# r4dl/LAENeRF

Hardware: AMD Instinct MI355X
Metric: Mrays/s, lego 800x800 train-step (4096 rays/step) (higher is better)
Workload: dtype f16 (table, MLP) / f32 (march, composite); 1 GPU; configs[1]: lego-like 800x800 pinhole rays, 4096 random pixels of one view per step, L=16 T=2^19 F=2 hash grid + 2x64 / 3x64 ffmlp, cascade 1, analytic occupancy (13% occupied), steady-state train step incl. backward + Adam; hip_graph_replay=True, march_pipelined_on_side_stream=True, steps_per_graph_replay=4, parallelism=1 independent ray-batch replicas (no data-path collective)

## Files before the change

### include/laenerf.h

```cpp
#ifndef LAENERF_H
#define LAENERF_H

#include <stdint.h>

#ifdef __cplusplus
extern "C" {
#endif

#if defined(__GNUC__) || defined(__clang__)
#define LAE_API __attribute__((visibility("default")))
#else
#define LAE_API
#endif

#define LAE_OK 0
#define LAE_EINVAL (-1)
#define LAE_ELAUNCH (-2)
#define LAE_ENULL (-3)

#define LAE_F32 0
#define LAE_F16 1

#define LAE_GRID_HASH 0
#define LAE_GRID_TILED 1
#define LAE_INTERP_LINEAR 0
#define LAE_INTERP_SMOOTHSTEP 1

#define LAE_ACT_RELU 0
#define LAE_ACT_EXPONENTIAL 1
#define LAE_ACT_SINE 2
#define LAE_ACT_SIGMOID 3
#define LAE_ACT_SQUAREPLUS 4
#define LAE_ACT_SOFTPLUS 5
#define LAE_ACT_NONE 6

#define LAE_ABI_TAG "abi16"
LAE_API const char* lae_version(void);
LAE_API const char* lae_last_error(void);


LAE_API int lae_near_far_from_aabb(const float* rays_o, const float* rays_d, const float* aabb,
                           uint32_t N, float min_near, float* nears, float* fars, void* stream);

LAE_API int lae_get_rays(const float* poses, uint32_t B, float fx, float fy, float cx, float cy, uint32_t H, uint32_t W,
                 const int64_t* inds, uint64_t inds_batch_stride, uint32_t N, int perturb, float off_x, float off_y,
                 float* rays_o, float* rays_d, const float* aabb, float min_near, float* nears, float* fars, void* stream);

#define LAE_IMG_U8 0
#define LAE_IMG_F16 1
#define LAE_IMG_F32 2
#define LAE_BATCH_IMAGE 0
#define LAE_BATCH_ALL 1
#define LAE_BG_WHITE 0
#define LAE_BG_RANDOM 1
LAE_API int lae_sample_train_batch(const void* images, int dtype, uint32_t n_img, uint32_t H, uint32_t W, uint32_t C,
                           const float* poses, float fx, float fy, float cx, float cy, uint32_t N,
                           const float* aabb, float min_near, uint64_t seed, int64_t* step_counter, int mode, int bg_mode,
                           int srgb_to_linear, float* rays_o, float* rays_d, float* nears, float* fars, float* gt,
                           float* bg_out, int64_t* inds, void* stream);
// ... 153 lines not shown
                                const int32_t* offsets_host, int32_t* nonfinite_flag, uint32_t* touched_lines, uint32_t* grad_dirty,
                                void* stream);

LAE_API uint64_t lae_grid_backward_plan_bytes(uint32_t B, uint32_t L);
LAE_API uint64_t lae_grid_touched_lines_words(uint64_t n_entries);
LAE_API int lae_grid_encode_backward_plan(const float* inputs, const int32_t* offsets, uint32_t B, uint32_t D, uint32_t C, uint32_t L,
                                  float S, uint32_t H, uint32_t gridtype, int align_corners, uint32_t interp, int dtype,
                                  float in_shift, float in_scale, const int32_t* offsets_host, void* plan,
                                  uint32_t* touched_lines, void* stream);
LAE_API int lae_grid_encode_backward_planned(const void* grad, const float* inputs, const int32_t* offsets, void* grad_embeddings,
                                     uint32_t B, uint32_t D, uint32_t C, uint32_t L, float S, uint32_t H, uint32_t gridtype,
                                     int align_corners, uint32_t interp, int dtype, float in_shift, float in_scale,
                                     const int32_t* offsets_host, const void* plan, int32_t* nonfinite_flag, uint32_t* grad_dirty,
                                     void* stream);

LAE_API uint64_t lae_grid_backward_workspace_bytes(uint32_t B, uint32_t L, int dtype);

LAE_API int lae_grid_forward_schedule(const int32_t* offsets_host, uint32_t L, float S, uint32_t H, uint32_t n_chunks,
                              uint32_t* nseg_out, uint32_t* segs_out);

LAE_API int lae_grid_set_forward_mode(int mode);

LAE_API int lae_grid_set_backward_mode(int mode);

LAE_API int lae_grad_total_variation(const void* inputs, const void* embeddings, void* grad,
                             const int32_t* offsets, float weight, uint32_t B, uint32_t D,
                             uint32_t C, uint32_t L, float S, uint32_t H, uint32_t gridtype,
                             int align_corners, int dtype, void* stream);


LAE_API int lae_sh_encode_forward(const float* inputs, float* outputs, uint32_t B, uint32_t D,
                          uint32_t C, float* dy_dx, void* stream);

LAE_API int lae_sh_encode_backward(const float* grad, const float* inputs, uint32_t B, uint32_t D,
                           uint32_t C, const float* dy_dx, float* grad_inputs, void* stream);


LAE_API int lae_ffmlp_forward(const void* inputs, const void* weights, uint32_t B, uint32_t input_dim,
                      uint32_t output_dim, uint32_t hidden_dim, uint32_t num_layers,
                      uint32_t activation, uint32_t output_activation, void* forward_buffer,
                      void* outputs, void* stream);

LAE_API int lae_ffmlp_inference(const void* inputs, const void* weights, uint32_t B, uint32_t input_dim,
                        uint32_t output_dim, uint32_t hidden_dim, uint32_t num_layers,
                        uint32_t activation, uint32_t output_activation, void* inference_buffer,
                        void* outputs, void* stream);
// ... 188 lines not shown
```

### laenerf_amd/_lib.py

```python
import ctypes
import os

import torch

_HERE = os.path.dirname(os.path.abspath(__file__))
SO_PATH = os.environ.get("LAE_HIP_LIB") or os.path.join(_HERE, "lib", "liblaenerf_hip.so")

u32, u64, f32, i32, vp = ctypes.c_uint32, ctypes.c_uint64, ctypes.c_float, ctypes.c_int, ctypes.c_void_p
i64, f64 = ctypes.c_int64, ctypes.c_double

SIGNATURES = {
    "lae_near_far_from_aabb": [vp, vp, vp, u32, f32, vp, vp, vp],
    "lae_sph_from_ray": [vp, vp, f32, u32, vp, vp],
    "lae_get_rays": [vp, u32, f32, f32, f32, f32, u32, u32, vp, u64, u32, i32, f32, f32, vp, vp, vp, f32, vp, vp, vp],
    "lae_morton3D": [vp, u32, vp, vp],
    "lae_morton3D_invert": [vp, u32, vp, vp],
    "lae_packbits": [vp, u32, f32, vp, vp],
    "lae_march_rays_train_scratch_bytes": [u32],
    "lae_march_rays_train": [vp, vp, vp, f32, f32, u32, u32, u32, u32, u32, vp, vp, vp, vp, vp, vp, vp, vp, vp, vp, vp],
    "lae_march_rays_train_limit": [vp, vp, vp, f32, f32, u32, u32, u32, u32, u32, vp, vp, vp, vp, vp, vp, vp, vp, vp, vp, vp, vp],
    "lae_sample_train_batch": [vp, i32, u32, u32, u32, u32, vp, f32, f32, f32, f32, u32, vp, f32, u64, vp, i32, i32, i32, vp, vp, vp, vp, vp,
                               vp, vp, vp],
    "lae_sample_train_batch_weighted": [vp, i32, u32, u32, u32, u32, vp, f32, f32, f32, f32, u32, vp, f32, u64, vp, i32, i32, vp, vp,
                                        vp, vp, vp, vp, vp, vp, vp, vp],
# ... 10 lines not shown
    "lae_march_rays": [u32, u32, vp, vp, vp, vp, f32, f32, u32, u32, u32, vp, vp, vp, vp, vp, vp, vp, vp],
    "lae_march_rays_distill": [u32, u32, vp, vp, vp, vp, f32, f32, u32, u32, u32, vp, vp, vp, vp, vp, vp, vp, vp, vp, vp],
    "lae_composite_rays": [u32, u32, f32, vp, vp, vp, vp, vp, vp, vp, vp, vp],
    "lae_composite_rays_distill": [u32, u32, f32, vp, vp, vp, vp, vp, vp, vp, vp, vp, vp, vp, vp],
    "lae_render_frame_workspace_bytes": [u32, u32, u64],
    "lae_render_frame_set_overlap": [i32],
    "lae_render_frame_mode": [],
    "lae_render_frame_last_status": [],
    "lae_render_frame_probe_us": [vp, u32],
    "lae_render_frame": [vp, vp, u32, vp, f32, vp, vp, f32, f32, u32, u32, u32, vp, vp, vp, u32, f32, u32, u32, i32, u32, vp, vp, f32, f32,
                         u32, u64, vp, vp, f32, f32, f32, i32, i32, vp, vp, vp, vp, vp, vp, u64, vp, vp],
    "lae_compact_scratch_bytes": [u32],
    "lae_compact_rays_alive": [vp, u32, vp, vp, vp, vp],
    "lae_grid_encode_forward": [vp, vp, vp, vp, u32, u32, u32, u32, f32, u32, vp, u32, i32, u32, i32, vp],
    "lae_grid_encode_backward": [vp, vp, vp, vp, vp, u32, u32, u32, u32, f32, u32, vp, vp, u32, i32, u32, i32, vp],
    "lae_grid_encode_forward_ex": [vp, vp, vp, vp, u32, u32, u32, u32, f32, u32, vp, u32, i32, u32, i32, i32, f32, f32, vp, vp],
    "lae_grid_encode_backward_ex": [vp, vp, vp, vp, vp, u32, u32, u32, u32, f32, u32, vp, vp, u32, i32, u32, i32, i32, f32, f32, vp, vp, vp, vp, vp],
    "lae_grid_backward_workspace_bytes": [u32, u32, i32],
    "lae_grid_backward_plan_bytes": [u32, u32],
    "lae_grid_touched_lines_words": [u64],
    "lae_grid_encode_backward_plan": [vp, vp, u32, u32, u32, u32, f32, u32, u32, i32, u32, i32, f32, f32, vp, vp, vp, vp],
    "lae_grid_encode_backward_planned": [vp, vp, vp, vp, u32, u32, u32, u32, f32, u32, u32, i32, u32, i32, f32, f32, vp, vp, vp, vp, vp],
    "lae_grid_set_backward_mode": [i32],
    "lae_grid_set_forward_mode": [i32],
    "lae_grid_forward_schedule": [vp, u32, f32, u32, u32, vp, vp],
    "lae_grad_total_variation": [vp, vp, vp, vp, f32, u32, u32, u32, u32, f32, u32, u32, i32, i32, vp],
    "lae_sh_encode_forward": [vp, vp, u32, u32, u32, vp, vp],
    "lae_sh_encode_backward": [vp, vp, u32, u32, u32, vp, vp, vp],
    "lae_freq_encode_forward": [vp, u32, u32, u32, u32, vp, vp],
    "lae_freq_encode_backward": [vp, vp, u32, u32, u32, u32, vp, vp],
    "lae_ffmlp_forward": [vp, vp, u32, u32, u32, u32, u32, u32, u32, vp, vp, vp],
    "lae_ffmlp_inference": [vp, vp, u32, u32, u32, u32, u32, u32, u32, vp, vp, vp],
    "lae_ffmlp_backward": [vp, vp, vp, vp, u32, u32, u32, u32, u32, u32, u32, i32, vp, vp, vp, vp],
    "lae_ffmlp_backward_ex": [vp, vp, vp, vp, u32, u32, u32, u32, u32, u32, u32, i32, vp, vp, vp, i32, vp, vp],
    "lae_nerf_head_forward": [vp, vp, vp, vp, u32, f32, vp, vp, vp, i32, vp],
    "lae_nerf_density_forward": [vp, vp, u32, f32, vp, vp, i32, vp],
    "lae_density_grid_positions": [vp, u32, u32, f32, vp, vp, vp, vp],
    "lae_density_grid_partial_scratch_bytes": [u32, u32],
    "lae_density_grid_partial_positions": [vp, u32, vp, vp, vp, u32, u32, f32, vp, vp, vp, vp, vp],
    "lae_density_grid_update": [vp, vp, u32, f32, f32, u32, vp, vp, vp],
    "lae_mark_untrained_grid": [vp, u32, f32, f32, f32, f32, u32, u32, f32, f32, i32, vp, vp],
    "lae_nerf_head_backward": [vp, vp, vp, vp, vp, vp, vp, vp, u32, f32, vp, vp, vp, vp, i32, i32, vp, vp, u32, u32, vp, vp, vp],
    "lae_nerf_field_backward": [vp, vp, vp, vp, vp, vp, vp, vp, u32, f32, vp, vp, vp, vp, i32, vp, vp, u32, u32, vp, vp,
                                vp, vp, vp, u32, f32, u32, u32, i32, u32, f32, f32, vp, vp, vp, vp, vp, vp],
    "lae_palette_forward": [vp, vp, vp, u32, u32, u32, vp, vp, vp, vp],
    "lae_palette_backward_scratch_bytes": [u32],
# ... 37 lines not shown
    "lae_workspace_bytes": [i32],
    "lae_version": [],
    "lae_last_error": [],
}
_RESTYPES = {
    "lae_march_rays_train_scratch_bytes": u64,
    "lae_compact_scratch_bytes": u64,
    "lae_density_grid_partial_scratch_bytes": u64,
    "lae_palette_backward_scratch_bytes": u64,
    "lae_style_loss_scratch_bytes": u64,
    "lae_recolor_compact_scratch_bytes": u64,
    "lae_marching_cubes_scratch_bytes": u64,
    "lae_style_image_scratch_bytes": u64,
    "lae_render_frame_workspace_bytes": u64,
    "lae_workspace_bytes": u64,
    "lae_grid_backward_workspace_bytes": u64,
    "lae_grid_backward_plan_bytes": u64,
    "lae_grid_touched_lines_words": u64,
    "lae_version": ctypes.c_char_p,
    "lae_last_error": ctypes.c_char_p,
}

_lib = None
ABI_TAG = b"abi16"


def _abi_of(path):
    lib = ctypes.CDLL(path)
    fn = lib.lae_version
    fn.argtypes, fn.restype = [], ctypes.c_char_p
    return lib, fn().split()[-1]


def load():
    global _lib
    if _lib is not None:
        return _lib
    if not os.path.exists(SO_PATH):
        raise RuntimeError(
            f"laenerf_amd: HIP library not built ({SO_PATH}); run `python -m laenerf_amd.build` "
            "(there is no CPU fallback)")
    if not os.environ.get("LAE_HIP_LIB"):
        from . import build as _build
        if _build.default_is_packed(SO_PATH):
            _build.build(force=True)
            if _build.default_is_packed(SO_PATH):
                raise RuntimeError(f"laenerf_amd: {SO_PATH} was built with packed-fp32 instructions and could not be rebuilt without them")
# ... 70 lines not shown
```

### laenerf_amd/backend.py

```python
import sys
import types

import numpy as np
import torch

from . import _lib
from ._lib import check, need_contig, need_cuda, ptr, stream

_F16 = torch.float16


def _dtype_code(t):
    if t.dtype == torch.float32:
        return 0
    if t.dtype == torch.float16:
        return 1
    raise RuntimeError(f"laenerf_amd: unsupported dtype {t.dtype} (float32 / float16 only)")


def _host_i32(a, n):
    if a is None:
        return None
    if not (isinstance(a, np.ndarray) and a.dtype == np.int32 and a.flags.c_contiguous and a.size == n):
        raise RuntimeError("laenerf_amd: offsets_host must be a contiguous int32 numpy array with L + 1 entries")
# ... 430 lines not shown
            check(lib.lae_grid_encode_backward_planned(ptr(grad), ptr(inputs), ptr(offsets), ptr(grad_embeddings), B, D, C, L, float(S), H,
                                                       gridtype, int(bool(align_corners)), interp, _dtype_code(grad), float(in_map[0]),
                                                       float(in_map[1]), _host_i32(offsets_host, L + 1), ptr(plan), nonfinite_flag, grad_dirty, stream()),
                  "grid_encode_backward")
            return
        args = (ptr(grad), ptr(inputs), ptr(embeddings), ptr(offsets), ptr(grad_embeddings), B, D, C, L, float(S), H,
                ptr(dy_dx), ptr(grad_inputs), gridtype, int(bool(align_corners)), interp, _dtype_code(grad))
        if (blc or tuple(in_map) != (0.0, 1.0) or offsets_host is not None or nonfinite_flag is not None or touched_lines is not None
                or grad_dirty is not None):
            check(lib.lae_grid_encode_backward_ex(*args, int(bool(blc)), float(in_map[0]), float(in_map[1]), _host_i32(offsets_host, L + 1),
                                                  nonfinite_flag, touched_lines, grad_dirty, stream()), "grid_encode_backward")
        else:
            check(lib.lae_grid_encode_backward(*args, stream()), "grid_encode_backward")

    @staticmethod
    def grid_backward_workspace_bytes(B, L, half=True):
        return int(_lib.load().lae_grid_backward_workspace_bytes(B, L, 1 if half else 0))

    @staticmethod
    def set_backward_mode(mode):
        check(_lib.load().lae_grid_set_backward_mode(int(mode)), "grid_set_backward_mode")

    @staticmethod
    def grad_total_variation(inputs, embeddings, grad, offsets, weight, B, D, C, L, S, H, gridtype, align_corners):
        need_cuda(inputs, embeddings, grad, offsets); need_contig(inputs, embeddings, grad, offsets)
        check(_lib.load().lae_grad_total_variation(ptr(inputs), ptr(embeddings), ptr(grad), ptr(offsets), float(weight), B, D,
                                                   C, L, float(S), H, gridtype, int(bool(align_corners)),
                                                   _dtype_code(embeddings), stream()), "grad_total_variation")


class _SHEncoder:
    @staticmethod
    def sh_encode_forward(inputs, outputs, B, D, C, dy_dx):
        need_cuda(inputs, outputs, dy_dx); need_contig(inputs, outputs, dy_dx)
        if inputs.dtype != torch.float32 or outputs.dtype != torch.float32:
            raise RuntimeError("sh_encode_forward: float32 required (sphere_harmonics.py:16 casts to fp32)")
        check(_lib.load().lae_sh_encode_forward(ptr(inputs), ptr(outputs), B, D, C, ptr(dy_dx), stream()), "sh_encode_forward")

    @staticmethod
    def sh_encode_backward(grad, inputs, B, D, C, dy_dx, grad_inputs):
        need_cuda(grad, inputs, dy_dx, grad_inputs); need_contig(grad, inputs, dy_dx, grad_inputs)
        if grad.dtype != torch.float32:
            raise RuntimeError("sh_encode_backward: float32 required")
        check(_lib.load().lae_sh_encode_backward(ptr(grad), ptr(inputs), B, D, C, ptr(dy_dx), ptr(grad_inputs), stream()),
              "sh_encode_backward")

# ... 350 lines not shown
        check(lib.lae_recolor_compact(ptr(depth), ptr(weights_sum), ptr(rays_o), ptr(rays_d), N, ptr(indices), ptr(slot_map), ptr(x_term),
                                      ptr(dirs), ptr(alpha), ptr(count), ptr(ws), stream()), "recolor_compact")

    @staticmethod
    def recolor_compose(slot_map, N, w_logits, o_raw, P, active_mask, palette, p_weights, p_bias, alpha, base, bg, mode, k, flags, out,
                        out_u8=None):
        ts = (slot_map, w_logits, o_raw, palette, p_weights, p_bias, alpha, base, bg, out, out_u8)
        need_cuda(*ts); need_contig(*ts)
        if w_logits.dtype != _F16 or o_raw.dtype != _F16 or slot_map.dtype != torch.int32 or (out_u8 is not None and out_u8.dtype != torch.uint8):
            raise RuntimeError("recolor_compose: logits / offsets float16, slot_map int32, out_u8 uint8")
        _need_f32(*(t for t in (palette, p_weights, p_bias, alpha, base, bg, out) if t is not None))
        if slot_map.numel() < N or out.numel() < 3 * N or (base is not None and base.numel() < 3 * N) or \
                (out_u8 is not None and out_u8.numel() < 3 * N) or bg.numel() < 3:
            raise RuntimeError("recolor_compose: a buffer is smaller than the view")
        check(_lib.load().lae_recolor_compose(ptr(slot_map), N, ptr(w_logits), w_logits.shape[1], ptr(o_raw), o_raw.shape[1], P, active_mask,
                                              ptr(palette), ptr(p_weights), ptr(p_bias), ptr(alpha), ptr(base), ptr(bg), int(mode), int(k),
                                              int(flags), ptr(out), ptr(out_u8), stream()), "recolor_compose")


style_backend = _Style

for _cls in (_RayMarching, _GridEncoder, _SHEncoder, _FFMLP):
    for _k, _v in list(vars(_cls).items()):
        if isinstance(_v, staticmethod) and not _k.startswith("_") and _k not in ("fused_backward_available", "ffmlp_set_mode", "set_backward_mode",
                                                                                   "allocate_splitk", "free_splitk", "render_frame_last_status",
                                                                                   "render_frame_check"):
            setattr(_cls, _k, staticmethod(_wrap_timed(_k, _v.__func__)))

raymarching_backend = _RayMarching
gridencoder_backend = _GridEncoder
shencoder_backend = _SHEncoder
ffmlp_backend = _FFMLP
freqencoder_backend = _FreqEncoder


def _as_module(name, cls):
    m = types.ModuleType(name)
    for k, v in vars(cls).items():
        if not k.startswith("_") and isinstance(v, staticmethod):
            setattr(m, k, v.__func__)
    m.__doc__ = f"laenerf_amd HIP backend standing in for the reference's `{name}` extension"
    return m


def install_as_reference_backends():
    _lib.load()
    for name, cls in (("_raymarching", _RayMarching), ("_gridencoder", _GridEncoder), ("_shencoder", _SHEncoder),
# ... 3 lines not shown
```

### laenerf_amd/csrc/gridencoder.hip

```cpp
#include <math.h>
#include <stdio.h>
#include <stdlib.h>
#include <algorithm>
#include <type_traits>
#include "lae_common.h"
#include "dw_reduce.h"
#include <vector>
#include <mutex>
#include <utility>

namespace {

constexpr int MAX_LEVELS = 32;
struct LevelScales { float scale[MAX_LEVELS]; float in_shift, in_scale; };

typedef _Float16 half_t;
typedef _Float16 half2_t __attribute__((ext_vector_type(2)));

__constant__ uint32_t k_primes[7] = {1u, 2654435761u, 805459861u, 3674653429u, 2097192037u, 1434869437u, 2165219737u};

#ifdef LAE_GRID_STAMPS
__device__ unsigned long long g_grid_stamps[32768 * 32];
#define GRID_STAMP(slot, i) do { if (threadIdx.x == 0 && (uint32_t)(i) < 32u) g_grid_stamps[(size_t)(slot) * 32 + (i)] = wall_clock64(); } while (0)
#define GRID_NOTE(slot, i, v) do { if (threadIdx.x == 0 && (uint32_t)(i) < 32u) g_grid_stamps[(size_t)(slot) * 32 + (i)] = (v); } while (0)
// ... 355 lines not shown
                    (__attribute__((address_space(1))) half2_t*)(tab + gi + ch), v);
            }
        } else {
#pragma unroll
            for (int ch = 0; ch < C; ch++) atomicAdd(tab + gi + ch, w * gc[ch]);
        }
    }
}

template <typename T> struct BVal;
template <> struct BVal<half_t> { using type = uint2; };
template <> struct BVal<float> { using type = float4; };
constexpr int FILL_THREADS = 256;
constexpr int SPT = 4;
constexpr int SEGS = 1;
constexpr uint32_t UNIT_SAMPLES = FILL_THREADS * SPT;
constexpr uint32_t STAGE_CAP = 4096 + 256;
constexpr uint32_t KEY_SINGLE = 15u;
constexpr int ACC_THREADS = 1024;
constexpr uint32_t BWD_MAX_SAMPLES = 1u << 24;
constexpr uint32_t COARSE_RES = 64;
constexpr bool WIDE_COARSE_UNITS = false;
constexpr uint32_t SUB_RECS = 64;
constexpr uint32_t TICKET_ARRIVALS = 2;
constexpr uint32_t TICKET_WORDS = TICKET_ARRIVALS + MAX_LEVELS * SUB_RECS;
template <typename T> constexpr uint32_t sub_rec_words() { return (sizeof(T) == 2 ? 2 * PART : PART) + PART / 64; }

struct BwdPlan {
    uint16_t* cnt;
    uint32_t* part_cnt;
    uint32_t* totals;
    uint32_t* offs;
    uint32_t* tickets;
};

__host__ __device__ __forceinline__ lae_dw::DwTailJob* plan_tail_job(const BwdPlan& plan) {
    static_assert((TICKET_WORDS * 4) % alignof(lae_dw::DwTailJob) == 0, "the tail job sits right behind the tickets");
    return reinterpret_cast<lae_dw::DwTailJob*>(plan.tickets + TICKET_WORDS);
}
__host__ __device__ __forceinline__ uint32_t* plan_dirty_snapshot(const BwdPlan& plan) {
    return plan.tickets + TICKET_WORDS + sizeof(lae_dw::DwTailJob) / 4;
}

__device__ __forceinline__ uint32_t pack_half2(float a, float b) {
    const half2_t h = {(half_t)a, (half_t)b};
    return __builtin_bit_cast(uint32_t, h);
// ... 381 lines not shown
}
__device__ __forceinline__ uint32_t fix24_to_half(long long t) {
    const uint32_t sign = t < 0 ? 0x8000u : 0u;
    const unsigned long long mag = t < 0 ? (unsigned long long)(-t) : (unsigned long long)t;
    if (mag < 1024ull) return sign | (uint32_t)mag;
    const int msb = 63 - __builtin_clzll(mag);
    const int shift = msb - 10;
    unsigned long long q = mag >> shift;
    if (shift > 0) {
        const unsigned long long rem = mag & ((1ull << shift) - 1ull), halfway = 1ull << (shift - 1);
        if (rem > halfway || (rem == halfway && (q & 1ull))) q++;
    }
    int e = msb - 9;
    if (q == 2048ull) { q = 1024ull; e++; }
    if (e >= 31) return sign | 0x7c00u;
    return sign | ((uint32_t)e << 10) | ((uint32_t)q & 1023u);
}
__device__ __forceinline__ bool half_nonfinite(uint32_t u) { return (u & 0x7c00u) == 0x7c00u; }

template <typename T>
__global__ __launch_bounds__(ACC_THREADS, 8) void k_bwd_acc(
    const int32_t* __restrict__ offsets, T* __restrict__ grad_grid, uint32_t L, LevelScales sc, uint32_t gridtype,
    bool align_corners, BwdPlan plan, const typename BVal<T>::type* __restrict__ qvals, const uint16_t* __restrict__ qkeys,
    unsigned long long* __restrict__ partials, int32_t* __restrict__ nf_flag, uint32_t bk_target) {
    using V = typename BVal<T>::type;
    constexpr bool HALF = sizeof(T) == 2;
    constexpr uint32_t ACCW = HALF ? 2 * PART : PART;
    __shared__ unsigned long long acc64[ACCW];
    __shared__ uint32_t poison[PART / 32];
    __shared__ uint32_t s_cnt[MAX_LEVELS], s_sub[MAX_LEVELS], s_first[MAX_LEVELS];
    __shared__ uint32_t s_ticket, s_arr;
    const uint32_t tid = threadIdx.x;
    if (tid < L) {
        const LevelBins lb = level_bins_of((uint32_t)(offsets[tid + 1] - offsets[tid]), bk_target);
        s_cnt[tid] = lb.P <= BK_MAX ? lb.P * lb.SUB : 0u;
        s_sub[tid] = lb.SUB;
    }
    __syncthreads();
    if (tid == 0) { uint32_t run = 0; for (uint32_t l = 0; l < L; l++) { s_first[l] = run; run += s_cnt[l]; } s_arr = run; }
    __syncthreads();
    const uint32_t total_buckets = s_arr;
    __syncthreads();

    auto apply = [&](uint32_t key, const V& v) {
        const uint32_t e0 = key & (PART - 1), code = key >> 12;
        const uint32_t e1 = e0 ^ ((2u << code) - 1u);
        if constexpr (HALF) {
            const uint32_t w0 = v.x, w1 = v.y;
            const uint32_t carry = (((w0 & 0x7c007c00u) + 0x28002800u) | ((w1 & 0x7c007c00u) + 0x28002800u)) & 0x80008000u;
            if (carry == 0) {
                long long a, b;
                half2_to_fix24_small(w0, a, b);
                atomicAdd(&acc64[e0], (unsigned long long)a);
                atomicAdd(&acc64[PART + e0], (unsigned long long)b);
// ... 2 lines not shown
                atomicAdd(&acc64[e1s], (unsigned long long)a);
                atomicAdd(&acc64[PART + e1s], (unsigned long long)b);
            } else {
                if (half_nonfinite(w0) || half_nonfinite(w0 >> 16)) atomicOr(&poison[e0 >> 5], 1u << (e0 & 31));
                else {
                    atomicAdd(&acc64[e0], (unsigned long long)half_to_fix24(w0 & 0xffffu));
                    atomicAdd(&acc64[PART + e0], (unsigned long long)half_to_fix24(w0 >> 16));
                }
                if (code != KEY_SINGLE) {
                    if (half_nonfinite(w1) || half_nonfinite(w1 >> 16)) atomicOr(&poison[e1 >> 5], 1u << (e1 & 31));
                    else {
                        atomicAdd(&acc64[e1], (unsigned long long)half_to_fix24(w1 & 0xffffu));
                        atomicAdd(&acc64[PART + e1], (unsigned long long)half_to_fix24(w1 >> 16));
                    }
                }
            }
        } else {
            float* af = reinterpret_cast<float*>(acc64);
            atomicAdd(af + e0, v.x); atomicAdd(af + PART + e0, v.y);
            if (code != KEY_SINGLE) { atomicAdd(af + e1, v.z); atomicAdd(af + PART + e1, v.w); }
        }
    };

    bool first_task = true;
    uint32_t tail_task;
    [[maybe_unused]] uint32_t stamp_task = 0;
    GRID_STAMP(4096 + blockIdx.x, 0);
    for (;;) {
        if (tid == 0) s_ticket = first_task ? blockIdx.x : atomicAdd(&plan.tickets[0], 1u) + gridDim.x;
        first_task = false;
        __syncthreads();
        const uint32_t t = __builtin_amdgcn_readfirstlane(s_ticket);
        GRID_STAMP(4096 + blockIdx.x, 1 + stamp_task * 6);
        if (t >= total_buckets) { tail_task = t - total_buckets; break; }
        GRID_NOTE(4096 + blockIdx.x, 2 + stamp_task * 6, t);
        const uint32_t item = t;
        uint32_t level = 0;
        while (level + 1 < L && item >= s_first[level + 1]) level++;
        level = __builtin_amdgcn_readfirstlane(level);
        const uint32_t bk = item - __builtin_amdgcn_readfirstlane(s_first[level]);
        const uint32_t SUB = __builtin_amdgcn_readfirstlane(s_sub[level]), p = bk / SUB, sub = bk % SUB;
        const uint32_t table_off = (uint32_t)offsets[level], hashmap_size = (uint32_t)offsets[level + 1] - table_off;
        const uint32_t n_raw = plan.totals[level * BK_MAX + p], q0_raw = plan.offs[level * BK_MAX + p], dirty_raw = *plan_dirty_snapshot(plan);
        const uint32_t n = __builtin_amdgcn_readfirstlane(n_raw), q0 = __builtin_amdgcn_readfirstlane(q0_raw);
        const bool grad_dirty = __builtin_amdgcn_readfirstlane(dirty_raw) != 0u;
        const uint32_t lo = (uint32_t)(((uint64_t)n * sub) / SUB), hi = (uint32_t)(((uint64_t)n * (sub + 1)) / SUB);
        if (n == 0) { __syncthreads(); continue; }
        const uint32_t part_lo = p << PART_SHIFT;
        const uint32_t n_ent = min(PART, hashmap_size - part_lo);
        T* __restrict__ dst = grad_grid + ((size_t)table_off + part_lo) * 2;
        uint32_t oldv[HALF ? PART / ACC_THREADS : 1];
        const uint32_t n_old = grad_dirty ? n_ent : 0u;
        if constexpr (HALF) {
#pragma unroll
            for (int it = 0; it < (int)(PART / ACC_THREADS); it++) { const uint32_t e = tid + it * ACC_THREADS; oldv[it] = e < n_old ? reinterpret_cast<const uint32_t*>(dst)[e] : 0u; }
        }
        for (uint32_t i = tid; i < ACCW; i += ACC_THREADS) acc64[i] = 0ull;
        if (tid < PART / 32) poison[tid] = 0u;
        __syncthreads();
        GRID_STAMP(4096 + blockIdx.x, 3 + stamp_task * 6);
        const uint32_t scale_res = (uint32_t)ceilf(sc.scale[level]) + 1;
        const V* __restrict__ pv = qvals + q0;
        const uint16_t* __restrict__ pk = qkeys + q0;
        if (!HALF && scale_res >= COARSE_RES) {
            uint32_t i = lo + tid;
            for (; i + 3 * ACC_THREADS < hi; i += 4 * ACC_THREADS) {
                V v[4]; uint32_t k[4];
#pragma unroll
                for (int j = 0; j < 4; j++) { v[j] = pv[i + j * ACC_THREADS]; k[j] = pk[i + j * ACC_THREADS]; }
#pragma unroll
                for (int j = 0; j < 4; j++) apply(k[j], v[j]);
            }
            for (; i < hi; i += ACC_THREADS) { const V v = pv[i]; const uint32_t k = pk[i]; apply(k, v); }
        } else {
            if constexpr (HALF) {
                using u4 = __attribute__((__vector_size__(16))) uint32_t;
                const uint32_t abs_lo = q0 + lo, abs_hi = q0 + hi, A0 = abs_lo & ~7u;
                const uint32_t n_groups = (abs_hi - A0 + 7u) >> 3;
                const __amdgpu_buffer_rsrc_t rs_v = __builtin_amdgcn_make_buffer_rsrc(const_cast<V*>(qvals + A0), 0, (int)(n_groups * 64u), 0x00020000);
                const __amdgpu_buffer_rsrc_t rs_k = __builtin_amdgcn_make_buffer_rsrc(const_cast<uint16_t*>(qkeys + A0), 0, (int)(n_groups * 16u), 0x00020000);
                const bool coarse = scale_res < COARSE_RES;
                for (uint32_t gq = coarse ? (tid & 63u) * (ACC_THREADS / 64) + (tid >> 6) : tid; gq < n_groups; gq += ACC_THREADS) {
                    const u4 va = __builtin_amdgcn_raw_buffer_load_b128(rs_v, (int)(gq * 64u), 0, 0);
                    const u4 vb = __builtin_amdgcn_raw_buffer_load_b128(rs_v, (int)(gq * 64u + 16u), 0, 0);
                    const u4 vc = __builtin_amdgcn_raw_buffer_load_b128(rs_v, (int)(gq * 64u + 32u), 0, 0);
                    const u4 vd = __builtin_amdgcn_raw_buffer_load_b128(rs_v, (int)(gq * 64u + 48u), 0, 0);
                    const u4 kk = __builtin_amdgcn_raw_buffer_load_b128(rs_k, (int)(gq * 16u), 0, 0);
                    const uint32_t w[16] = {va[0], va[1], va[2], va[3], vb[0], vb[1], vb[2], vb[3], vc[0], vc[1], vc[2], vc[3], vd[0], vd[1], vd[2], vd[3]};
                    const uint32_t a0 = A0 + gq * 8u;
                    const uint32_t first = a0 < abs_lo ? abs_lo - a0 : 0u, last = min(8u, abs_hi - a0);
                    if (!coarse) {
#pragma unroll
                        for (int j = 0; j < 8; j++)
                            if ((uint32_t)j >= first && (uint32_t)j < last) { V v; v.x = w[2 * j]; v.y = w[2 * j + 1]; apply((kk[j >> 1] >> (16 * (j & 1))) & 0xffffu, v); }
                        continue;
                    }
                    uint32_t ckey = 0;
                    long long s00 = 0, s01 = 0, s10 = 0, s11 = 0;
                    bool bad0 = false, bad1 = false, started = false;
                    auto flush = [&]() {
                        const uint32_t e0 = ckey & (PART - 1), code = ckey >> 12;
                        const uint32_t e1 = e0 ^ ((2u << code) - 1u);
                        if (bad0) atomicOr(&poison[e0 >> 5], 1u << (e0 & 31));
                        else { atomicAdd(&acc64[e0], (unsigned long long)s00); atomicAdd(&acc64[PART + e0], (unsigned long long)s01); }
                        if (code != KEY_SINGLE) {
                            if (bad1) atomicOr(&poison[e1 >> 5], 1u << (e1 & 31));
                            else { atomicAdd(&acc64[e1], (unsigned long long)s10); atomicAdd(&acc64[PART + e1], (unsigned long long)s11); }
                        }
                    };
#pragma unroll
// ... 12 lines not shown
                                half2_to_fix24_small(w1, a, b); s10 += a; s11 += b;
                            } else {
                                if (half_nonfinite(w0) || half_nonfinite(w0 >> 16)) bad0 = true;
                                else { s00 += half_to_fix24(w0 & 0xffffu); s01 += half_to_fix24(w0 >> 16); }
                                if (half_nonfinite(w1) || half_nonfinite(w1 >> 16)) bad1 = true;
                                else { s10 += half_to_fix24(w1 & 0xffffu); s11 += half_to_fix24(w1 >> 16); }
                            }
                        }
                    }
                    if (started) flush();
                }
            } else {
                for (uint32_t c = lo + tid * 8u; c < hi; c += ACC_THREADS * 8u) {
                    V v[8]; uint32_t k[8];
#pragma unroll
                    for (int j = 0; j < 8; j++) { const uint32_t ii = min(c + (uint32_t)j, hi - 1u); v[j] = pv[ii]; k[j] = pk[ii]; }
                    const uint32_t cnt = min(8u, hi - c);
#pragma unroll
                    for (int j = 0; j < 8; j++) if ((uint32_t)j < cnt) apply(k[j], v[j]);
                }
            }
        }
        GRID_STAMP(4096 + blockIdx.x, 4 + stamp_task * 6);
        __syncthreads();
        GRID_STAMP(4096 + blockIdx.x, 5 + stamp_task * 6);
        if (SUB > 1) {
            unsigned long long* __restrict__ rec = partials + (size_t)(level * SUB_RECS + p) * sub_rec_words<T>();
            uint32_t* __restrict__ rec_poison = reinterpret_cast<uint32_t*>(rec + ACCW);
            if constexpr (HALF) {
                for (uint32_t i = tid; i < ACCW; i += ACC_THREADS) { const unsigned long long v = acc64[i]; if (v) atomicAdd(rec + i, v); }
            } else {
                const float* af = reinterpret_cast<const float*>(acc64);
                float* rf = reinterpret_cast<float*>(rec);
                for (uint32_t i = tid; i < 2 * PART; i += ACC_THREADS) { const float v = af[i]; if (v != 0.0f) atomicAdd(rf + i, v); }
            }
            if (tid < PART / 32 && poison[tid]) atomicOr(rec_poison + tid, poison[tid]);
            asm volatile("s_waitcnt vmcnt(0)" ::: "memory");
            __syncthreads();
            if (tid == 0) s_arr = atomicAdd(&plan.tickets[TICKET_ARRIVALS + level * SUB_RECS + p], 1u);
            __syncthreads();
            if (s_arr != SUB - 1) { GRID_STAMP(4096 + blockIdx.x, 6 + stamp_task * 6); stamp_task++; __syncthreads(); continue; }
            for (uint32_t i = tid; i < ACCW; i += ACC_THREADS) acc64[i] = atomicExch(rec + i, 0ull);
            if (tid < PART / 32) poison[tid] = atomicExch(rec_poison + tid, 0u);
            __syncthreads();
        }
        if constexpr (HALF) {
            uint32_t* d2 = reinterpret_cast<uint32_t*>(dst);
            bool wrote_nonfinite = false;
#pragma unroll
            for (int it = 0; it < (int)(PART / ACC_THREADS); it++) {
                const uint32_t e = tid + it * ACC_THREADS;
                if (e >= n_ent) break;
                const long long i0 = (long long)acc64[e], i1 = (long long)acc64[PART + e];
                const bool bad = (poison[(tid >> 5) + it * (ACC_THREADS / 32)] >> (tid & 31)) & 1u;
                if (i0 == 0 && i1 == 0 && !bad) continue;
                const uint32_t o = oldv[it];
                uint32_t r0, r1;
                if (bad) { r0 = 0x7e00u; r1 = 0x7e00u; }
                else {
                    r0 = half_nonfinite(o) ? (o & 0xffffu) : fix24_to_half(i0 + half_to_fix24(o & 0xffffu));
                    r1 = half_nonfinite(o >> 16) ? (o >> 16) : fix24_to_half(i1 + half_to_fix24(o >> 16));
                }
                d2[e] = r0 | (r1 << 16);
                wrote_nonfinite |= half_nonfinite(r0) || half_nonfinite(r1);
            }
            if (nf_flag && wrote_nonfinite) atomicOr(nf_flag, 1);
        } else {
            const float* af = reinterpret_cast<const float*>(acc64);
            float2* d2 = reinterpret_cast<float2*>(dst);
            for (uint32_t e = tid; e < n_ent; e += ACC_THREADS) {
                const float v0 = af[e], v1 = af[PART + e];
                if (v0 == 0.0f && v1 == 0.0f) continue;
                float2 o = d2[e]; o.x += v0; o.y += v1; d2[e] = o;
                if (nf_flag && !(isfinite(o.x) && isfinite(o.y))) atomicOr(nf_flag, 1);
            }
        }
        GRID_STAMP(4096 + blockIdx.x, 6 + stamp_task * 6);
        stamp_task++;
        __syncthreads();
    }
    static_assert(sizeof(acc64) >= lae_dw::DWR_LDS_FLOATS * sizeof(float) && ACC_THREADS == (int)lae_dw::DWR_THREADS, "tail tasks run in this workgroup");
    const lae_dw::DwTailJob& tail = *plan_tail_job(plan);
    const uint32_t n_tail = __builtin_amdgcn_readfirstlane(tail.n_tasks);
    while (tail_task < n_tail) {
        lae_dw::dw_tail_task(tail, tail_task, reinterpret_cast<float*>(acc64));
        if (tid == 0) s_ticket = atomicAdd(&plan.tickets[0], 1u) + gridDim.x;
        __syncthreads();
        tail_task = __builtin_amdgcn_readfirstlane(s_ticket) - total_buckets;
    }
}

template <typename T>
__global__ __launch_bounds__(256) void k_out_transpose(const T* __restrict__ in, T* __restrict__ out, uint32_t B, uint32_t L) {
    using V = typename std::conditional<sizeof(T) == 2, uint32_t, uint2>::type;
    __shared__ V tile[256 * 33];
// ... 427 lines not shown
    uint8_t* ex = ws + merge_bytes() + plan_bytes;
    const size_t cap = (size_t)L * U * UNIT_SAMPLES * 8;
    V* qvals = reinterpret_cast<V*>(ex);
    uint16_t* qkeys = reinterpret_cast<uint16_t*>(ex + up(cap * sizeof(V)));
    const T* g = (const T*)gT;
    T* ge = (T*)gemb;
    if (!caller_plan) bwd_plan<T>(inputs, offsets, B, L, a, plan);
    const lae_dw::DwTailJob tail_job = a.tail ? *a.tail : lae_dw::DwTailJob{};
#ifdef LAE_GRID_BWD_PHASE_PROBE
    const char* phase_env = getenv("LAE_GRID_BWD_PHASE");
    const int phase_probe = phase_env ? atoi(phase_env) : 0;
    if (phase_probe != 2)
#endif
    if (a.gridtype == 0 && !a.align && a.interp == 0)
        k_bwd_walk<T, true, true><<<U / SEGS * L, FILL_THREADS, 0, a.stream>>>(g, inputs, offsets, B, L, a.sc, a.gridtype, a.align, a.interp, U, plan, qvals, qkeys, nullptr, nullptr, a.dirty, tail_job);
    else
        k_bwd_walk<T, true, false><<<U / SEGS * L, FILL_THREADS, 0, a.stream>>>(g, inputs, offsets, B, L, a.sc, a.gridtype, a.align, a.interp, U, plan, qvals, qkeys, nullptr, nullptr, a.dirty, tail_job);
#ifdef LAE_GRID_BWD_PHASE_PROBE
    if (phase_probe == 1) return lae::check_launch("grid backward (fill-only probe)");
#endif
    static const uint32_t bk_env = [] { const char* e = getenv("LAE_GRID_BWD_BK_TARGET"); return e ? (uint32_t)std::min(std::max(atoi(e), 1), (int)SUB_RECS) : 0u; }();
    static_assert(BK_TARGET <= SUB_RECS && 64u <= SUB_RECS, "bk_target choices must fit the merge records");
    const uint32_t bk_target = std::min(bk_env ? bk_env : (B >= 400000u ? 64u : BK_TARGET), SUB_RECS);
    k_bwd_acc<T><<<(uint32_t)lae::num_cus() * 2, ACC_THREADS, 0, a.stream>>>(offsets, ge, L, a.sc, a.gridtype, a.align, plan, qvals, qkeys, partials, a.nf_flag, bk_target);
    bool need_generic = true;
    if (a.offsets_host) {
        need_generic = false;
        for (uint32_t l = 0; l < L; l++)
            if (!level_is_binned((uint32_t)(a.offsets_host[l + 1] - a.offsets_host[l]))) need_generic = true;
    }
    if (need_generic) {
        const uint32_t nbg = lae::cdiv(B, GRID_BLOCK);
        k_grid_bwd<T, 3, 2><<<nbg * L, GRID_BLOCK, 0, a.stream>>>(g, inputs, offsets, ge, B, L, a.sc, a.gridtype, a.align, a.interp, nbg,
                                                                  (L % 8) == 0, 2, (uint64_t)B * 2, true);
    }
    return LAE_OK;
}

static inline size_t touched_words(const int32_t* offsets_host, uint32_t L) { return ((size_t)offsets_host[L] >> 3 >> 5) + 2; }

static int g_force_atomic_bwd = 0;

static int grid_backward(const void* grad, const float* inputs, const void* embeddings, const int32_t* offsets,
                         void* grad_embeddings, uint32_t B, uint32_t D, uint32_t C, uint32_t L, float S, uint32_t H,
                         const void* dy_dx, void* grad_inputs, uint32_t gridtype, int align_corners, uint32_t interp,
                         int dtype, bool blc, void* stream, float in_shift = 0.0f, float in_scale = 1.0f,
                         const int32_t* offsets_host = nullptr, const void* plan = nullptr, int32_t* nf_flag = nullptr,
// ... 213 lines not shown
    const uint32_t per_xcd = fwd_sched_build(fs, L, n_chunks, sc, offsets_host);
    for (int x = 0; x < 8; x++) {
        nseg_out[x] = fs.nseg[x];
        for (uint32_t q = 0; q < fs.nseg[x]; q++) {
            uint32_t* o = segs_out + ((size_t)x * FWD_MAX_SEG + q) * 3;
            o[0] = fs.seg[x][q].level; o[1] = fs.seg[x][q].c0; o[2] = fs.seg[x][q].n;
        }
    }
    return (int)per_xcd;
}

int lae_grid_set_forward_mode(int mode) {
    if (mode < 0 || mode > 2) return LAE_EINVAL;
    g_fwd_mode = mode;
    return LAE_OK;
}

int lae_grid_set_backward_mode(int mode) {
    if (mode != 0 && mode != 1) return LAE_EINVAL;
    g_force_atomic_bwd = mode;
    return LAE_OK;
}

int lae_grad_total_variation(const void* inputs, const void* embeddings, void* grad, const int32_t* offsets,
                             float weight, uint32_t B, uint32_t D, uint32_t C, uint32_t L, float S, uint32_t H,
                             uint32_t gridtype, int align_corners, int dtype, void* stream) {
    if (B == 0) return LAE_OK;
    if (!inputs || !embeddings || !grad || !offsets) return LAE_ENULL;
    if (dtype != LAE_F32 || gridtype > 1) return LAE_EINVAL;
    LevelScales sc;
    int rc = fill_scales(sc, L, S, H);
    if (rc) return rc;
    hipStream_t s = reinterpret_cast<hipStream_t>(stream);
    const bool al = align_corners != 0;
    const float* in = (const float*)inputs; const float* e = (const float*)embeddings; float* g = (float*)grad;
    switch (D) {
        case 2: rc = tv_c<2>(in, e, g, offsets, weight, B, C, L, sc, gridtype, al, s); break;
        case 3: rc = tv_c<3>(in, e, g, offsets, weight, B, C, L, sc, gridtype, al, s); break;
        case 4: rc = tv_c<4>(in, e, g, offsets, weight, B, C, L, sc, gridtype, al, s); break;
        case 5: rc = tv_c<5>(in, e, g, offsets, weight, B, C, L, sc, gridtype, al, s); break;
        default: rc = LAE_EINVAL;
    }
    if (rc) return rc;
    return lae::check_launch("grad_total_variation");
}

// ... 9 lines not shown
```

Before: 11.65 Mrays/s.

## Prefetch next ticket and plan in grid backward accumulator, zero LDS on drain

The persistent hash-grid backward accumulation kernel now draws its next work ticket and loads that bucket's plan totals and offsets while the current bucket is still being processed. The next bucket is posted through shared memory, which removes the serialized atomic-ticket, sync and plan-load round trip between tasks. Shared accumulators are zeroed once up front and then cleared during the merge and write-out passes, so the separate zero-and-barrier step per task goes away. The level lookup uses a wave ballot instead of a linear scan. The old serial path stays available behind an environment variable or API toggle. The changes add complexity around barrier placement and the correctness of the zero-on-drain logic.

Result: no change. 11.67 Mrays/s (median of 4 runs) (+0.2%).

```diff
diff --git a/include/laenerf.h b/include/laenerf.h
--- a/include/laenerf.h
+++ b/include/laenerf.h
@@ -34,7 +34,7 @@
 #define LAE_ACT_SOFTPLUS 5
 #define LAE_ACT_NONE 6
 
-#define LAE_ABI_TAG "abi16"
+#define LAE_ABI_TAG "abi17"
 LAE_API const char* lae_version(void);
 LAE_API const char* lae_last_error(void);
 
@@ -234,6 +234,8 @@
 LAE_API int lae_grid_set_forward_mode(int mode);
 
 LAE_API int lae_grid_set_backward_mode(int mode);
+
+LAE_API int lae_grid_set_backward_serial_tasks(int on);
 
 LAE_API int lae_grad_total_variation(const void* inputs, const void* embeddings, void* grad,
                              const int32_t* offsets, float weight, uint32_t B, uint32_t D,
diff --git a/laenerf_amd/_lib.py b/laenerf_amd/_lib.py
--- a/laenerf_amd/_lib.py
+++ b/laenerf_amd/_lib.py
@@ -56,6 +56,7 @@
     "lae_grid_encode_backward_plan": [vp, vp, u32, u32, u32, u32, f32, u32, u32, i32, u32, i32, f32, f32, vp, vp, vp, vp],
     "lae_grid_encode_backward_planned": [vp, vp, vp, vp, u32, u32, u32, u32, f32, u32, u32, i32, u32, i32, f32, f32, vp, vp, vp, vp, vp],
     "lae_grid_set_backward_mode": [i32],
+    "lae_grid_set_backward_serial_tasks": [i32],
     "lae_grid_set_forward_mode": [i32],
     "lae_grid_forward_schedule": [vp, u32, f32, u32, u32, vp, vp],
     "lae_grad_total_variation": [vp, vp, vp, vp, f32, u32, u32, u32, u32, f32, u32, u32, i32, i32, vp],
@@ -139,7 +140,7 @@
 }
 
 _lib = None
-ABI_TAG = b"abi16"
+ABI_TAG = b"abi17"
 
 
 def _abi_of(path):
diff --git a/laenerf_amd/backend.py b/laenerf_amd/backend.py
--- a/laenerf_amd/backend.py
+++ b/laenerf_amd/backend.py
@@ -476,6 +476,10 @@
         check(_lib.load().lae_grid_set_backward_mode(int(mode)), "grid_set_backward_mode")
 
     @staticmethod
+    def set_backward_serial_tasks(on):
+        check(_lib.load().lae_grid_set_backward_serial_tasks(int(bool(on))), "grid_set_backward_serial_tasks")
+
+    @staticmethod
     def grad_total_variation(inputs, embeddings, grad, offsets, weight, B, D, C, L, S, H, gridtype, align_corners):
         need_cuda(inputs, embeddings, grad, offsets); need_contig(inputs, embeddings, grad, offsets)
         check(_lib.load().lae_grad_total_variation(ptr(inputs), ptr(embeddings), ptr(grad), ptr(offsets), float(weight), B, D,
@@ -872,7 +876,7 @@
 
 for _cls in (_RayMarching, _GridEncoder, _SHEncoder, _FFMLP):
     for _k, _v in list(vars(_cls).items()):
-        if isinstance(_v, staticmethod) and not _k.startswith("_") and _k not in ("fused_backward_available", "ffmlp_set_mode", "set_backward_mode",
+        if isinstance(_v, staticmethod) and not _k.startswith("_") and _k not in ("fused_backward_available", "ffmlp_set_mode", "set_backward_mode", "set_backward_serial_tasks",
                                                                                    "allocate_splitk", "free_splitk", "render_frame_last_status",
                                                                                    "render_frame_check"):
             setattr(_cls, _k, staticmethod(_wrap_timed(_k, _v.__func__)))
diff --git a/laenerf_amd/csrc/gridencoder.hip b/laenerf_amd/csrc/gridencoder.hip
--- a/laenerf_amd/csrc/gridencoder.hip
+++ b/laenerf_amd/csrc/gridencoder.hip
@@ -401,6 +401,12 @@
 constexpr uint32_t COARSE_RES = 64;
 constexpr bool WIDE_COARSE_UNITS = false;
 constexpr uint32_t SUB_RECS = 64;
+constexpr uint32_t ACC_SERIAL_TASKS = 1u << 31;
+int g_acc_serial_tasks = -1;
+inline bool acc_serial_tasks() {
+    if (g_acc_serial_tasks < 0) { const char* e = getenv("LAE_GRID_BWD_SERIAL_TASKS"); g_acc_serial_tasks = e && e[0] == '1' ? 1 : 0; }
+    return g_acc_serial_tasks == 1;
+}
 constexpr uint32_t TICKET_ARRIVALS = 2;
 constexpr uint32_t TICKET_WORDS = TICKET_ARRIVALS + MAX_LEVELS * SUB_RECS;
 template <typename T> constexpr uint32_t sub_rec_words() { return (sizeof(T) == 2 ? 2 * PART : PART) + PART / 64; }
@@ -828,14 +834,17 @@
 __global__ __launch_bounds__(ACC_THREADS, 8) void k_bwd_acc(
     const int32_t* __restrict__ offsets, T* __restrict__ grad_grid, uint32_t L, LevelScales sc, uint32_t gridtype,
     bool align_corners, BwdPlan plan, const typename BVal<T>::type* __restrict__ qvals, const uint16_t* __restrict__ qkeys,
-    unsigned long long* __restrict__ partials, int32_t* __restrict__ nf_flag, uint32_t bk_target) {
+    unsigned long long* __restrict__ partials, int32_t* __restrict__ nf_flag, uint32_t bk_target_flags) {
     using V = typename BVal<T>::type;
     constexpr bool HALF = sizeof(T) == 2;
+    const bool serial = (bk_target_flags & ACC_SERIAL_TASKS) != 0u;
+    const uint32_t bk_target = bk_target_flags & ~ACC_SERIAL_TASKS;
     constexpr uint32_t ACCW = HALF ? 2 * PART : PART;
     __shared__ unsigned long long acc64[ACCW];
     __shared__ uint32_t poison[PART / 32];
     __shared__ uint32_t s_cnt[MAX_LEVELS], s_sub[MAX_LEVELS], s_first[MAX_LEVELS];
     __shared__ uint32_t s_ticket, s_arr;
+    __shared__ uint32_t s_next[3];
     const uint32_t tid = threadIdx.x;
     if (tid < L) {
         const LevelBins lb = level_bins_of((uint32_t)(offsets[tid + 1] - offsets[tid]), bk_target);
@@ -884,42 +893,95 @@
         }
     };
 
+    auto zero64 = [&](uint32_t i) {
+        uint32_t z;
+        asm volatile("v_mov_b32 %0, 0" : "=v"(z));
+        acc64[i] = ((unsigned long long)z << 32) | z;
+    };
+    auto level_of = [&](uint32_t item) -> uint32_t {
+        const uint32_t lane = tid & 63u;
+        static_assert(MAX_LEVELS <= 64, "one lane per level");
+        return (uint32_t)__popcll(__ballot(lane < L && item >= s_first[lane])) - 1u;
+    };
+    uint32_t n_raw = 0, q0_raw = 0;
+    auto request_plan = [&](uint32_t tk) {
+        if (tk < total_buckets) {
+            const uint32_t lv = level_of(tk);
+            const uint32_t pp = (tk - __builtin_amdgcn_readfirstlane(s_first[lv])) / __builtin_amdgcn_readfirstlane(s_sub[lv]);
+            n_raw = plan.totals[lv * BK_MAX + pp]; q0_raw = plan.offs[lv * BK_MAX + pp];
+        }
+    };
+    const bool grad_dirty = __builtin_amdgcn_readfirstlane(*plan_dirty_snapshot(plan)) != 0u;
+    for (uint32_t i = tid; i < ACCW; i += ACC_THREADS) acc64[i] = 0ull;
+    if (tid < PART / 32) poison[tid] = 0u;
     bool first_task = true;
+    uint32_t t = blockIdx.x;
     uint32_t tail_task;
     [[maybe_unused]] uint32_t stamp_task = 0;
     GRID_STAMP(4096 + blockIdx.x, 0);
+    uint32_t nx_t = 0;
+    auto request_next = [&](uint32_t tk) { if (tid < 64u) { nx_t = tk; n_raw = q0_raw = 0u; request_plan(tk); } };
+    auto post_next = [&]() { if (tid == 0) { s_next[0] = nx_t; s_next[1] = n_raw; s_next[2] = q0_raw; } };
+    if (!serial) { request_next(t); post_next(); }
+    __syncthreads();
     for (;;) {
-        if (tid == 0) s_ticket = first_task ? blockIdx.x : atomicAdd(&plan.tickets[0], 1u) + gridDim.x;
-        first_task = false;
-        __syncthreads();
-        const uint32_t t = __builtin_amdgcn_readfirstlane(s_ticket);
+        if (serial) {
+            if (!first_task) {
+                if (tid == 0) s_ticket = atomicAdd(&plan.tickets[0], 1u) + gridDim.x;
+                __syncthreads();
+                t = __builtin_amdgcn_readfirstlane(s_ticket);
+            }
+            request_plan(t);
+        } else {
+            t = __builtin_amdgcn_readfirstlane(s_next[0]);
+            n_raw = s_next[1]; q0_raw = s_next[2];
+        }
         GRID_STAMP(4096 + blockIdx.x, 1 + stamp_task * 6);
         if (t >= total_buckets) { tail_task = t - total_buckets; break; }
         GRID_NOTE(4096 + blockIdx.x, 2 + stamp_task * 6, t);
+        constexpr uint32_t NOT_DRAWN = 0xffffffffu;
+        uint32_t next_ticket = serial ? 0u : NOT_DRAWN;
+        auto draw_next = [&]() {
+            if (tid == 0 && next_ticket == NOT_DRAWN) {
+                uint32_t zero;
+                asm volatile("v_mov_b32 %0, 0" : "=v"(zero));
+                next_ticket = atomicAdd(plan.tickets + zero, 1u);
+            }
+        };
+        auto next_in_hand = [&]() {
+            if (tid < 64u) { draw_next(); request_next(__builtin_amdgcn_readfirstlane(next_ticket) + gridDim.x); }
+        };
         const uint32_t item = t;
-        uint32_t level = 0;
-        while (level + 1 < L && item >= s_first[level + 1]) level++;
-        level = __builtin_amdgcn_readfirstlane(level);
+        const uint32_t level = level_of(item);
         const uint32_t bk = item - __builtin_amdgcn_readfirstlane(s_first[level]);
         const uint32_t SUB = __builtin_amdgcn_readfirstlane(s_sub[level]), p = bk / SUB, sub = bk % SUB;
         const uint32_t table_off = (uint32_t)offsets[level], hashmap_size = (uint32_t)offsets[level + 1] - table_off;
-        const uint32_t n_raw = plan.totals[level * BK_MAX + p], q0_raw = plan.offs[level * BK_MAX + p], dirty_raw = *plan_dirty_snapshot(plan);
         const uint32_t n = __builtin_amdgcn_readfirstlane(n_raw), q0 = __builtin_amdgcn_readfirstlane(q0_raw);
-        const bool grad_dirty = __builtin_amdgcn_readfirstlane(dirty_raw) != 0u;
         const uint32_t lo = (uint32_t)(((uint64_t)n * sub) / SUB), hi = (uint32_t)(((uint64_t)n * (sub + 1)) / SUB);
-        if (n == 0) { __syncthreads(); continue; }
+        if (n == 0) {
+            if (serial) { first_task = false; __syncthreads(); continue; }
+            __syncthreads();
+            next_in_hand(); post_next();
+            __syncthreads();
+            continue;
+        }
         const uint32_t part_lo = p << PART_SHIFT;
         const uint32_t n_ent = min(PART, hashmap_size - part_lo);
         T* __restrict__ dst = grad_grid + ((size_t)table_off + part_lo) * 2;
         uint32_t oldv[HALF ? PART / ACC_THREADS : 1];
         const uint32_t n_old = grad_dirty ? n_ent : 0u;
         if constexpr (HALF) {
-#pragma unroll
-            for (int it = 0; it < (int)(PART / ACC_THREADS); it++) { const uint32_t e = tid + it * ACC_THREADS; oldv[it] = e < n_old ? reinterpret_cast<const uint32_t*>(dst)[e] : 0u; }
-        }
-        for (uint32_t i = tid; i < ACCW; i += ACC_THREADS) acc64[i] = 0ull;
-        if (tid < PART / 32) poison[tid] = 0u;
-        __syncthreads();
+            uint32_t e0 = tid;
+            asm volatile("" : "+v"(e0));
+#pragma unroll
+            for (int it = 0; it < (int)(PART / ACC_THREADS); it++) { const uint32_t e = e0 + it * ACC_THREADS; oldv[it] = e < n_old ? reinterpret_cast<const uint32_t*>(dst)[e] : 0u; }
+        }
+        if (serial && !first_task) {
+            for (uint32_t i = tid; i < ACCW; i += ACC_THREADS) acc64[i] = 0ull;
+            if (tid < PART / 32) poison[tid] = 0u;
+            __syncthreads();
+        }
+        first_task = false;
         GRID_STAMP(4096 + blockIdx.x, 3 + stamp_task * 6);
         const uint32_t scale_res = (uint32_t)ceilf(sc.scale[level]) + 1;
         const V* __restrict__ pv = qvals + q0;
@@ -948,6 +1010,7 @@
                     const u4 vc = __builtin_amdgcn_raw_buffer_load_b128(rs_v, (int)(gq * 64u + 32u), 0, 0);
                     const u4 vd = __builtin_amdgcn_raw_buffer_load_b128(rs_v, (int)(gq * 64u + 48u), 0, 0);
                     const u4 kk = __builtin_amdgcn_raw_buffer_load_b128(rs_k, (int)(gq * 16u), 0, 0);
+                    draw_next();
                     const uint32_t w[16] = {va[0], va[1], va[2], va[3], vb[0], vb[1], vb[2], vb[3], vc[0], vc[1], vc[2], vc[3], vd[0], vd[1], vd[2], vd[3]};
                     const uint32_t a0 = A0 + gq * 8u;
                     const uint32_t first = a0 < abs_lo ? abs_lo - a0 : 0u, last = min(8u, abs_hi - a0);
@@ -1006,38 +1069,58 @@
             }
         }
         GRID_STAMP(4096 + blockIdx.x, 4 + stamp_task * 6);
+        if (!serial) next_in_hand();
         __syncthreads();
         GRID_STAMP(4096 + blockIdx.x, 5 + stamp_task * 6);
+        if (!serial) post_next();
         if (SUB > 1) {
             unsigned long long* __restrict__ rec = partials + (size_t)(level * SUB_RECS + p) * sub_rec_words<T>();
             uint32_t* __restrict__ rec_poison = reinterpret_cast<uint32_t*>(rec + ACCW);
+            uint32_t i0 = tid;
+            asm volatile("" : "+v"(i0));
             if constexpr (HALF) {
-                for (uint32_t i = tid; i < ACCW; i += ACC_THREADS) { const unsigned long long v = acc64[i]; if (v) atomicAdd(rec + i, v); }
+                for (uint32_t i = i0; i < ACCW; i += ACC_THREADS) { const unsigned long long v = acc64[i]; if (v) { atomicAdd(rec + i, v); zero64(i); } }
             } else {
-                const float* af = reinterpret_cast<const float*>(acc64);
+                float* af = reinterpret_cast<float*>(acc64);
                 float* rf = reinterpret_cast<float*>(rec);
-                for (uint32_t i = tid; i < 2 * PART; i += ACC_THREADS) { const float v = af[i]; if (v != 0.0f) atomicAdd(rf + i, v); }
-            }
-            if (tid < PART / 32 && poison[tid]) atomicOr(rec_poison + tid, poison[tid]);
+                for (uint32_t i = i0; i < 2 * PART; i += ACC_THREADS) {
+                    const float v = af[i];
+                    if (__float_as_uint(v) != 0u) af[i] = 0.0f;
+                    if (v != 0.0f) atomicAdd(rf + i, v);
+                }
+            }
+            if (tid < PART / 32) { const uint32_t pw = poison[tid]; if (pw) { atomicOr(rec_poison + tid, pw); poison[tid] = 0u; } }
             asm volatile("s_waitcnt vmcnt(0)" ::: "memory");
             __syncthreads();
             if (tid == 0) s_arr = atomicAdd(&plan.tickets[TICKET_ARRIVALS + level * SUB_RECS + p], 1u);
             __syncthreads();
-            if (s_arr != SUB - 1) { GRID_STAMP(4096 + blockIdx.x, 6 + stamp_task * 6); stamp_task++; __syncthreads(); continue; }
-            for (uint32_t i = tid; i < ACCW; i += ACC_THREADS) acc64[i] = atomicExch(rec + i, 0ull);
+            if (s_arr != SUB - 1) {
+                GRID_STAMP(4096 + blockIdx.x, 6 + stamp_task * 6); stamp_task++;
+                if (serial) __syncthreads();
+                continue;
+            }
+            for (uint32_t i = i0; i < ACCW; i += ACC_THREADS) acc64[i] = atomicExch(rec + i, 0ull);
             if (tid < PART / 32) poison[tid] = atomicExch(rec_poison + tid, 0u);
             __syncthreads();
         }
         if constexpr (HALF) {
             uint32_t* d2 = reinterpret_cast<uint32_t*>(dst);
             bool wrote_nonfinite = false;
+            uint32_t badbits = 0;
+#pragma unroll
+            for (int it = 0; it < (int)(PART / ACC_THREADS); it++) badbits |= ((poison[(tid >> 5) + it * (ACC_THREADS / 32)] >> (tid & 31)) & 1u) << it;
+            if ((tid & 31u) == 0u) {
+#pragma unroll
+                for (int it = 0; it < (int)(PART / ACC_THREADS); it++) poison[(tid >> 5) + it * (ACC_THREADS / 32)] = 0u;
+            }
 #pragma unroll
             for (int it = 0; it < (int)(PART / ACC_THREADS); it++) {
                 const uint32_t e = tid + it * ACC_THREADS;
-                if (e >= n_ent) break;
                 const long long i0 = (long long)acc64[e], i1 = (long long)acc64[PART + e];
-                const bool bad = (poison[(tid >> 5) + it * (ACC_THREADS / 32)] >> (tid & 31)) & 1u;
+                const bool bad = (badbits >> it) & 1u;
                 if (i0 == 0 && i1 == 0 && !bad) continue;
+                zero64(e); zero64(PART + e);
+                if (e >= n_ent) continue;
                 const uint32_t o = oldv[it];
                 uint32_t r0, r1;
                 if (bad) { r0 = 0x7e00u; r1 = 0x7e00u; }
@@ -1050,11 +1133,12 @@
             }
             if (nf_flag && wrote_nonfinite) atomicOr(nf_flag, 1);
         } else {
-            const float* af = reinterpret_cast<const float*>(acc64);
+            float* af = reinterpret_cast<float*>(acc64);
             float2* d2 = reinterpret_cast<float2*>(dst);
-            for (uint32_t e = tid; e < n_ent; e += ACC_THREADS) {
+            for (uint32_t e = tid; e < PART; e += ACC_THREADS) {
                 const float v0 = af[e], v1 = af[PART + e];
-                if (v0 == 0.0f && v1 == 0.0f) continue;
+                if ((__float_as_uint(v0) | __float_as_uint(v1)) != 0u) { af[e] = 0.0f; af[PART + e] = 0.0f; }
+                if (e >= n_ent || (v0 == 0.0f && v1 == 0.0f)) continue;
                 float2 o = d2[e]; o.x += v0; o.y += v1; d2[e] = o;
                 if (nf_flag && !(isfinite(o.x) && isfinite(o.y))) atomicOr(nf_flag, 1);
             }
@@ -1528,7 +1612,8 @@
     static const uint32_t bk_env = [] { const char* e = getenv("LAE_GRID_BWD_BK_TARGET"); return e ? (uint32_t)std::min(std::max(atoi(e), 1), (int)SUB_RECS) : 0u; }();
     static_assert(BK_TARGET <= SUB_RECS && 64u <= SUB_RECS, "bk_target choices must fit the merge records");
     const uint32_t bk_target = std::min(bk_env ? bk_env : (B >= 400000u ? 64u : BK_TARGET), SUB_RECS);
-    k_bwd_acc<T><<<(uint32_t)lae::num_cus() * 2, ACC_THREADS, 0, a.stream>>>(offsets, ge, L, a.sc, a.gridtype, a.align, plan, qvals, qkeys, partials, a.nf_flag, bk_target);
+    k_bwd_acc<T><<<(uint32_t)lae::num_cus() * 2, ACC_THREADS, 0, a.stream>>>(offsets, ge, L, a.sc, a.gridtype, a.align, plan, qvals, qkeys, partials, a.nf_flag,
+                                                                              bk_target | (acc_serial_tasks() ? ACC_SERIAL_TASKS : 0u));
     bool need_generic = true;
     if (a.offsets_host) {
         need_generic = false;
@@ -1788,6 +1873,12 @@
     return LAE_OK;
 }
 
+int lae_grid_set_backward_serial_tasks(int on) {
+    if (on != 0 && on != 1) return LAE_EINVAL;
+    g_acc_serial_tasks = on;
+    return LAE_OK;
+}
+
 int lae_grad_total_variation(const void* inputs, const void* embeddings, void* grad, const int32_t* offsets,
                              float weight, uint32_t B, uint32_t D, uint32_t C, uint32_t L, float S, uint32_t H,
                              uint32_t gridtype, int align_corners, int dtype, void* stream) {
```
